# vita-epfl/motion-style-transfer

Hardware: AMD Instinct MI355X
Metric: trajectories/sec fwd+bwd (Y-Net+LoRA, SDD shortterm) (higher is better)
Workload: dtype f32; 1 GPU; C2: SDD shortterm Y-Net + LoRA rank=1 on encoder[0-4], 256x256 raster, obs=8 pred=12; batch_per_gpu=32, global_batch=32, raster=256x256, obs_len=8, pred_len=12, train_net=mosa_1, parallelism=dp1, trainable_floats=8190

## Files before the change

### motion-style-transfer_amd/csrc/wgrad_mfma.hip

```cpp
#include "ynet_common.h"
#include "../../include/ynet_hip.h"
#include <type_traits>
#include <stdlib.h>
#include <stdio.h>

struct WgradArgs {
    YSrc src[YNET_MAX_SRC];
    int nsrc, cin;
    const float* dy;
    long long dy_bs;
    const float* mask;
    long long mask_bs;
    float* partial_w;
    float* partial_b;
    int B, H, W, cout;
    int tiles_x, tiles_y, ntiles, nsplit, co_blks, ci_blks;
    int seg, nseg_y, nsegs;
    int debug;
#ifdef YNET_WG_PROFILE
    unsigned long long* prof;
#endif
};

template <int KS>
// ... 504 lines not shown
#endif
    for (; tile < a.ntiles; tile += a.nsplit) {
#ifdef YNET_WG_PROFILE
        const unsigned long long p0 = __builtin_amdgcn_s_memtime();
#endif
        asm volatile("s_waitcnt vmcnt(0)" ::: "memory");
#ifdef YNET_WG_PROFILE
        const unsigned long long p1 = __builtin_amdgcn_s_memtime();
#endif
        __syncthreads();
#ifdef YNET_WG_PROFILE
        const unsigned long long p2 = __builtin_amdgcn_s_memtime();
#endif
        if (tile + a.nsplit < a.ntiles) issue(next_tile(), buf ^ 1);
#ifdef YNET_WG_PROFILE
        const unsigned long long p3 = __builtin_amdgcn_s_memtime();
#endif
        compute(buf);
#ifdef YNET_WG_PROFILE
        const unsigned long long p4 = __builtin_amdgcn_s_memtime();
        pw += p1 - p0; pb += p2 - p1; pi += p3 - p2; pc += p4 - p3;
#endif
        buf ^= 1;
    }
#ifdef YNET_WG_PROFILE
    if (lane == 0) {
        unsigned long long* pr = a.prof;
        atomicAdd(pr + 0, __builtin_amdgcn_s_memtime() - pt0);
        atomicAdd(pr + 1, pw); atomicAdd(pr + 2, pb); atomicAdd(pr + 3, pi); atomicAdd(pr + 4, pc); atomicAdd(pr + 5, 1ull);
        atomicAdd(pr + 6, prof_dma);
    }
#endif

    if (rpN > 1) {
        float* red = smem;
        __syncthreads();
        if (rp > 0) {
            float* w = red + (wave - cbN * ibN) * 37 * 64 + lane;
#pragma unroll
            for (int t = 0; t < KK; ++t)
#pragma unroll
                for (int e = 0; e < 4; ++e) w[(t * 4 + e) * 64] = acc[t][e];
            w[36 * 64] = bsum;
        }
        __syncthreads();
        if (rp == 0) {
            for (int q = 1; q < rpN; ++q) {
                const float* w = red + (cb + cbN * (ib + ibN * q) - cbN * ibN) * 37 * 64 + lane;
#pragma unroll
                for (int t = 0; t < KK; ++t)
#pragma unroll
                    for (int e = 0; e < 4; ++e) acc[t][e] += w[(t * 4 + e) * 64];
                bsum += w[36 * 64];
            }
        }
    }
    if (rp == 0) {
        float* pw = a.partial_w + (long long)split * a.cout * a.cin * KK;
        const int ci = ib * 16 + r16;
#pragma unroll
        for (int e = 0; e < 4; ++e) {
            const int co = cb * 16 + 4 * kq + e;
            if (co < nco && ci < ncib) {
#pragma unroll
                for (int t = 0; t < KK; ++t) pw[((long long)(co0 + co) * a.cin + ci0 + ci) * KK + t] = acc[t][e];
            }
        }
        if (want_bias && ib == 0) {
            float v = bsum;
            v += __shfl_xor(v, 16);
            v += __shfl_xor(v, 32);
            const int co = cb * 16 + r16;
            if (kq == 0 && co < nco) a.partial_b[(long long)split * a.cout + co0 + co] = v;
        }
    }
}

typedef float f32x2 __attribute__((ext_vector_type(2)));
template <int OFF>
__device__ __forceinline__ void wg_ld2(f32x2& v, unsigned addr) {
    asm volatile("ds_read_b64 %0, %1 offset:%2" : "=v"(v) : "v"(addr), "n"(OFF));
}

template <bool MASK>
struct WgRollCfg {
    static constexpr int TW = 32, XCS = 44, XRS = 32 * XCS, XPS = 2 * XRS, XRING = 3 * XPS;
    static constexpr int PQ = 2 * 32 * 11;
    static constexpr int XI = (PQ + 255) / 256;
    static constexpr int DDATA = 2 * TW / 4, DQ = (DDATA + 1 + 6) / 8 * 8 + 1, DCH = DQ * 4;
    static constexpr int DS = 32 * DCH + 128, DBUF = DS * (MASK ? 2 : 1);
    static constexpr int DI = (32 * DQ + 255) / 256;
    static constexpr int LDS_FLOATS = XRING + 2 * DBUF, LDS_BYTES = LDS_FLOATS * 4;
    static constexpr int NGRP = 8;
    static_assert(DCH % 32 == 4 && (XCS * 4) % 16 == 0, "operand strides");
    static_assert(3 * 37 * 64 <= LDS_FLOATS, "cross-wave reduction scratch fits");
};

template <bool MASK>
__global__ __launch_bounds__(256, MASK ? 2 : 3) void wgrad_roll_kernel(const WgradArgs a) {
    using C = WgRollCfg<MASK>;
    constexpr int TW = C::TW, XCS = C::XCS, XRS = C::XRS, XPS = C::XPS, DQ = C::DQ, DCH = C::DCH, XI = C::XI, DI = C::DI, KK = 9;
    extern __shared__ __attribute__((aligned(16))) float smem[];
    auto ds_of = [&](int b) { return smem + C::XRING + b * C::DBUF; };
    auto ms_of = [&](int b) { return smem + C::XRING + b * C::DBUF + C::DS; };

    const int tid = threadIdx.x, lane = tid & 63;
    const int wave = __builtin_amdgcn_readfirstlane(tid >> 6);
    const int r16 = lane & 15, kq = lane >> 4;
    int bid = blockIdx.x;
    const int cib = bid % a.ci_blks;
    bid /= a.ci_blks;
    const int cob = bid % a.co_blks;
    const int split = bid / a.co_blks;
    const int H = a.H, W = a.W;
    const int HW = __builtin_amdgcn_readfirstlane(H * W);
    const unsigned plane_bytes = (unsigned)HW * 4u;
    const int ci0 = cib * 32, co0 = cob * 32;
    const int ncib = min(32, a.cin - ci0), nco = min(32, a.cout - co0);
    const bool want_bias = (a.partial_b != nullptr) && cib == 0;
    const int cbN = nco > 16 ? 2 : 1, ibN = ncib > 16 ? 2 : 1, rpN = 4 / (cbN * ibN);
    const int cb = wave % cbN, ib = (wave / cbN) % ibN, rp = wave / (cbN * ibN);

    int xsrc[XI], xrow[XI], xcol[XI];
    unsigned xcoff[XI];
#pragma unroll
    for (int k = 0; k < XI; ++k) {
        const int q = tid + k * 256;
        const int row = q / 352, within = q - row * 352, ch = within / 11, u = within - ch * 11;
        xrow[k] = row;
        xcol[k] = 4 * u - 4;
        int c = ci0 + ch, sid = -1;
        unsigned off = 0;
        if (q < C::PQ && u < 10 && ch < ncib) {
#pragma unroll
            for (int s = 0; s < YNET_MAX_SRC; ++s) {
                if (sid < 0 && s < a.nsrc) {
                    if (c < a.src[s].c) {
                        sid = s;
                        off = (unsigned)c * plane_bytes;
                    } else {
                        c -= a.src[s].c;
                    }
                }
            }
        }
        xsrc[k] = sid;
        xcoff[k] = off;
    }
    unsigned xs_in[XI], xs_l[XI], xs_r[XI], xs_lr[XI];
#pragma unroll
    for (int k = 0; k < XI; ++k) {
        const bool ok = xsrc[k] >= 0;
        const unsigned in = ok ? xcoff[k] + (unsigned)(xrow[k] * W + xcol[k] + 4) * 4u : 0x80000000u;
        const bool lh = xcol[k] < 0, rh = xcol[k] >= TW;
        xs_in[k] = in;
        xs_l[k] = lh ? 0x80000000u : in;
        xs_r[k] = rh ? 0x80000000u : in;
        xs_lr[k] = (lh || rh) ? 0x80000000u : in;
    }
    unsigned dstat[DI];
#pragma unroll
    for (int k = 0; k < DI; ++k) {
        const int q = tid + k * 256;
        const int ch = q / DQ, within = q - ch * DQ;
        const bool ok = q < 32 * DQ && within < C::DDATA;
        dstat[k] = ok ? (unsigned)ch * plane_bytes + (unsigned)((within / (TW / 4)) * W + (within % (TW / 4)) * 4) * 4u : 0x80000000u;
    }

    typedef const __attribute__((address_space(4))) WgradArgs* wg_kargs_t;
    auto issue_pair = [&](int b, int x0, int m, int slot) {
        wg_kargs_t ka = (wg_kargs_t)__builtin_amdgcn_kernarg_segment_ptr();
        asm volatile("" : "+s"(ka));
        float* xs = smem + slot * XPS;
        const int y0 = 2 * m - 1;
        const bool at_left = x0 == 0, at_right = x0 + TW >= W;
        unsigned xo[XI], xso;
        if (y0 >= 0 && y0 + 1 < H && y0 * W + x0 - 4 >= 0) {
            xso = (unsigned)(y0 * W + x0 - 4) * 4u;
            if (!at_left && !at_right) {
#pragma unroll
                for (int k = 0; k < XI; ++k) xo[k] = xs_in[k];
            } else {
#pragma unroll
                for (int k = 0; k < XI; ++k) {
                    const unsigned l = at_right ? xs_lr[k] : xs_l[k];
                    xo[k] = at_left ? l : xs_r[k];
                }
            }
        } else {
            xso = 0u;
#pragma unroll
            for (int k = 0; k < XI; ++k) {
                const int gy = y0 + xrow[k], gx = x0 + xcol[k];
                const bool ok = xsrc[k] >= 0 && gy >= 0 && gy < H && gx >= 0 && gx < W;
                xo[k] = ok ? xcoff[k] + (unsigned)(gy * W + gx) * 4u : 0x80000000u;
            }
        }
        const int nsrc = ka->nsrc;
        if (nsrc == 1) {
            const __amdgpu_buffer_rsrc_t r = __builtin_amdgcn_make_buffer_rsrc(
                const_cast<float*>(ka->src[0].p + (long long)b * ka->src[0].bs), 0, (unsigned)ka->src[0].c * plane_bytes, 0x00020000);
#pragma unroll
            for (int k = 0; k < XI - 1; ++k) wg_dma16s(r, xs + (k * 256 + wave * 64) * 4, xo[k], xso);
            if (wave < 3) wg_dma16s(r, xs + ((XI - 1) * 256 + wave * 64) * 4, xo[XI - 1], xso);
        } else {
#pragma unroll 1
            for (int s = 0; s < nsrc; ++s) {
                const __amdgpu_buffer_rsrc_t r = __builtin_amdgcn_make_buffer_rsrc(
                    const_cast<float*>(ka->src[s].p + (long long)b * ka->src[s].bs), 0, (unsigned)ka->src[s].c * plane_bytes, 0x00020000);
#pragma unroll
                for (int k = 0; k < XI; ++k)
                    if (xsrc[k] == s) wg_dma16s(r, xs + (k * 256 + wave * 64) * 4, xo[k], xso);
            }
        }
    };
    auto issue_dy = [&](int b, int x0, int j, int buf) {
        wg_kargs_t ka = (wg_kargs_t)__builtin_amdgcn_kernarg_segment_ptr();
        asm volatile("" : "+s"(ka));
        constexpr int DFULL = 32 * DQ / 256;
        static_assert(32 * DQ - DFULL * 256 <= 64, "the partial instruction fits one wave");
        const unsigned dso = (unsigned)(2 * j * W + x0) * 4u;
        {
            const __amdgpu_buffer_rsrc_t r = __builtin_amdgcn_make_buffer_rsrc(
                const_cast<float*>(ka->dy + (long long)b * ka->dy_bs + (long long)co0 * HW), 0, (unsigned)nco * plane_bytes, 0x00020000);
            float* ds = ds_of(buf);
#pragma unroll
            for (int k = 0; k < DFULL; ++k) wg_dma16s(r, ds + (k * 256 + wave * 64) * 4, dstat[k], dso);
            if (DI > DFULL && wave == 0) wg_dma16s(r, ds + (DFULL * 256) * 4, dstat[DI - 1], dso);
        }
        if (MASK) {
            const __amdgpu_buffer_rsrc_t r = __builtin_amdgcn_make_buffer_rsrc(
                const_cast<float*>(ka->mask + (long long)b * ka->mask_bs + (long long)co0 * HW), 0, (unsigned)nco * plane_bytes, 0x00020000);
            float* ms = ms_of(buf);
#pragma unroll
            for (int k = 0; k < DFULL; ++k) wg_dma16s(r, ms + (k * 256 + wave * 64) * 4, dstat[k], dso);
            if (DI > DFULL && wave == 0) wg_dma16s(r, ms + (DFULL * 256) * 4, dstat[DI - 1], dso);
        }
    };

    f32x4 acc[KK];
#pragma unroll
    for (int i = 0; i < KK; ++i) acc[i] = f32x4{0.f, 0.f, 0.f, 0.f};

    const unsigned x_lane = (unsigned)(size_t)(wg_lds_ptr_t)(smem + (ib * 16 + r16) * XCS + 2 * kq + 2) + 32u * rp;
    const unsigned d_lane = (unsigned)(size_t)(wg_lds_ptr_t)(smem + C::XRING + (cb * 16 + r16) * DCH + 2 * kq) + 32u * rp;
    f32x2 bsum2 = f32x2{0.f, 0.f};
    auto compute = [&](auto rpn_tag, int buf, unsigned sa, unsigned sb) {
        constexpr int RPN = decltype(rpn_tag)::value, NG = C::NGRP / RPN;
        const unsigned ab = d_lane + (unsigned)(buf * C::DBUF * 4), mb = ab + C::DS * 4;
        unsigned pa[4];
        pa[0] = x_lane + sa;
        pa[1] = x_lane + sa + XRS * 4;
        pa[2] = x_lane + sb;
        pa[3] = x_lane + sb + XRS * 4;
        f32x2 av[2], mv[2], q[2][KK];
        mv[0] = mv[1] = f32x2{1.f, 1.f};
        auto rd = [&](auto g_tag, f32x2& a_, f32x2& m_, f32x2* q_) {
            constexpr int G = decltype(g_tag)::value, r = G >> 2, col = (G & 3) * 32;
            wg_ld2<32 * G>(a_, ab);
            if (MASK) wg_ld2<32 * G>(m_, mb);
            wg_ld2<col>(q_[0], pa[r]);
            wg_ld2<col + 8>(q_[1], pa[r]);
            wg_ld2<col + 16>(q_[2], pa[r]);
            wg_ld2<col>(q_[3], pa[r + 1]);
            wg_ld2<col + 8>(q_[4], pa[r + 1]);
            wg_ld2<col + 16>(q_[5], pa[r + 1]);
            wg_ld2<col>(q_[6], pa[r + 2]);
            wg_ld2<col + 8>(q_[7], pa[r + 2]);
            wg_ld2<col + 16>(q_[8], pa[r + 2]);
        };
        auto lds_wait = []() { asm volatile("s_waitcnt lgkmcnt(0)" ::: "memory"); };
        auto select = [&](f32x2& a_, const f32x2& m_) {
            if (MASK) {
                a_.x = m_.x > 0.f ? a_.x : 0.f;
                a_.y = m_.y > 0.f ? a_.y : 0.f;
            }
        };
        auto mfmas = [&](const f32x2& a_c, const f32x2* q_c) {
#pragma unroll
            for (int ky = 0; ky < 3; ++ky) {
                acc[ky * 3 + 0] = __builtin_amdgcn_mfma_f32_16x16x4f32(a_c.x, q_c[ky * 3 + 0].y, acc[ky * 3 + 0], 0, 0, 0);
                acc[ky * 3 + 1] = __builtin_amdgcn_mfma_f32_16x16x4f32(a_c.x, q_c[ky * 3 + 1].x, acc[ky * 3 + 1], 0, 0, 0);
                acc[ky * 3 + 2] = __builtin_amdgcn_mfma_f32_16x16x4f32(a_c.x, q_c[ky * 3 + 1].y, acc[ky * 3 + 2], 0, 0, 0);
            }
#pragma unroll
            for (int ky = 0; ky < 3; ++ky) {
                acc[ky * 3 + 0] = __builtin_amdgcn_mfma_f32_16x16x4f32(a_c.y, q_c[ky * 3 + 1].x, acc[ky * 3 + 0], 0, 0, 0);
                acc[ky * 3 + 1] = __builtin_amdgcn_mfma_f32_16x16x4f32(a_c.y, q_c[ky * 3 + 1].y, acc[ky * 3 + 1], 0, 0, 0);
                acc[ky * 3 + 2] = __builtin_amdgcn_mfma_f32_16x16x4f32(a_c.y, q_c[ky * 3 + 2].x, acc[ky * 3 + 2], 0, 0, 0);
            }
        };
        rd(std::integral_constant<int, 0>{}, av[0], mv[0], q[0]);
        lds_wait();
        select(av[0], mv[0]);
        auto groups = [&](auto self, auto i_tag) -> void {
            constexpr int I = decltype(i_tag)::value, cur = I & 1, nxt = cur ^ 1;
#ifdef YNET_WG_EXPERIMENT
            if constexpr (I + 1 < NG) if (!(a.debug & 4)) rd(std::integral_constant<int, (I + 1) * RPN>{}, av[nxt], mv[nxt], q[nxt]);
#else
            if constexpr (I + 1 < NG) rd(std::integral_constant<int, (I + 1) * RPN>{}, av[nxt], mv[nxt], q[nxt]);
#endif
            __builtin_amdgcn_sched_barrier(0);
            mfmas(av[cur], q[cur]);
            __builtin_amdgcn_sched_barrier(0);
            if constexpr (I + 1 < NG) {
                lds_wait();
                select(av[nxt], mv[nxt]);
            }
            bsum2 += av[cur];
            __builtin_amdgcn_sched_barrier(0);
            if constexpr (I + 1 < NG) self(self, std::integral_constant<int, I + 1>{});
        };
        groups(groups, std::integral_constant<int, 0>{});
    };

    const int seg = a.seg, nseg_y = a.nseg_y, tiles_x = a.tiles_x, tiles_y = a.tiles_y;
    bool first = true;
    for (int sidx = split; sidx < a.nsegs; sidx += a.nsplit) {
        const int xt = sidx % tiles_x, t2 = sidx / tiles_x;
        const int ys = t2 % nseg_y, b = t2 / nseg_y;
        const int x0 = xt * TW, j0 = ys * seg, j1 = min(j0 + seg, tiles_y);
        if (!first) __syncthreads();
        first = false;
        issue_pair(b, x0, j0, 0);
        issue_pair(b, x0, j0 + 1, 1);
        issue_dy(b, x0, j0, 0);
        int sj = 0, buf = 0;
        for (int j = j0; j < j1; ++j) {
            asm volatile("s_waitcnt vmcnt(0)" ::: "memory");
            __syncthreads();
            const int s1 = sj == 2 ? 0 : sj + 1, s2 = s1 == 2 ? 0 : s1 + 1;
            if (j + 1 < j1 && !(a.debug & 1)) {
                issue_pair(b, x0, j + 2, s2);
                issue_dy(b, x0, j + 1, buf ^ 1);
            }
            if (!(a.debug & 2)) {
                const unsigned sa = (unsigned)(sj * XPS * 4), sb = (unsigned)(s1 * XPS * 4);
                if (rpN == 1) compute(std::integral_constant<int, 1>{}, buf, sa, sb);
                else if (rpN == 2) compute(std::integral_constant<int, 2>{}, buf, sa, sb);
                else compute(std::integral_constant<int, 4>{}, buf, sa, sb);
            }
            buf ^= 1;
            sj = s1;
        }
    }

    float bsum = bsum2.x + bsum2.y;
    if (rpN > 1) {
        float* red = smem;
        __syncthreads();
        if (rp > 0) {
            float* w = red + (wave - cbN * ibN) * 37 * 64 + lane;
#pragma unroll
            for (int t = 0; t < KK; ++t)
#pragma unroll
                for (int e = 0; e < 4; ++e) w[(t * 4 + e) * 64] = acc[t][e];
            w[36 * 64] = bsum2.x + bsum2.y;
        }
        __syncthreads();
        if (rp == 0) {
            for (int q = 1; q < rpN; ++q) {
                const float* w = red + (cb + cbN * (ib + ibN * q) - cbN * ibN) * 37 * 64 + lane;
#pragma unroll
                for (int t = 0; t < KK; ++t)
#pragma unroll
                    for (int e = 0; e < 4; ++e) acc[t][e] += w[(t * 4 + e) * 64];
                bsum += w[36 * 64];
            }
        }
    }
    if (rp == 0) {
        float* pw = a.partial_w + (long long)split * a.cout * a.cin * KK;
        const int ci = ib * 16 + r16;
#pragma unroll
        for (int e = 0; e < 4; ++e) {
            const int co = cb * 16 + 4 * kq + e;
            if (co < nco && ci < ncib) {
#pragma unroll
                for (int t = 0; t < KK; ++t) pw[((long long)(co0 + co) * a.cin + ci0 + ci) * KK + t] = acc[t][e];
            }
        }
        if (want_bias && ib == 0) {
            float v = bsum;
            v += __shfl_xor(v, 16);
            v += __shfl_xor(v, 32);
            const int co = cb * 16 + r16;
            if (kq == 0 && co < nco) a.partial_b[(long long)split * a.cout + co0 + co] = v;
        }
    }
}

struct Wg1x1Args {
    const float* x;
    long long x_bs;
    const float* dy;
    long long dy_bs;
    float* partial_w;
    float* partial_b;
    int B, cout, HW, hw16;
    long long chunks;
};

template <int CT>
__global__ __launch_bounds__(256) void wgrad1x1_stream_kernel(const Wg1x1Args a) {
    __shared__ float red[3][CT * 2 * 4 + CT][64];
    const int lane = threadIdx.x & 63, wave = threadIdx.x >> 6, r16 = lane & 15, kq = lane >> 4;
    f32x4 acc[CT][2];
    float bs[CT];
#pragma unroll
    for (int t = 0; t < CT; ++t) {
        acc[t][0] = acc[t][1] = f32x4{0.f, 0.f, 0.f, 0.f};
        bs[t] = 0.f;
    }
    const long long stride = (long long)gridDim.x * 4;
    long long c = (long long)blockIdx.x * 4 + wave;
    int b = (int)(c / a.hw16), pc = (int)(c - (long long)b * a.hw16);
    const int sb = (int)(stride / a.hw16), sp = (int)(stride - (long long)sb * a.hw16);
    const long long HW = a.HW;
    auto load = [&](int bb, int pp, f32x4& xa, f32x4& xb, f32x4* d) {
        const float* xp = a.x + (long long)bb * a.x_bs + (long long)r16 * HW + pp * 16 + 4 * kq;
        xa = *reinterpret_cast<const f32x4*>(xp);
        xb = *reinterpret_cast<const f32x4*>(xp + 16 * HW);
        const float* dp = a.dy + (long long)bb * a.dy_bs + (long long)r16 * HW + pp * 16 + 4 * kq;
#pragma unroll
        for (int t = 0; t < CT; ++t)
            d[t] = (t * 16 + r16 < a.cout) ? *reinterpret_cast<const f32x4*>(dp + (long long)t * 16 * HW) : f32x4{0.f, 0.f, 0.f, 0.f};
    };
    f32x4 xa, xb, d[CT], nxa, nxb, nd[CT];
    if (c < a.chunks) load(b, pc, xa, xb, d);
    while (c < a.chunks) {
        const long long cn = c + stride;
        int bn = b + sb, pn = pc + sp;
        if (pn >= a.hw16) {
            pn -= a.hw16;
            ++bn;
        }
        if (cn < a.chunks) load(bn, pn, nxa, nxb, nd);
#pragma unroll
        for (int e = 0; e < 4; ++e)
#pragma unroll
            for (int t = 0; t < CT; ++t) {
                acc[t][0] = __builtin_amdgcn_mfma_f32_16x16x4f32(d[t][e], xa[e], acc[t][0], 0, 0, 0);
                acc[t][1] = __builtin_amdgcn_mfma_f32_16x16x4f32(d[t][e], xb[e], acc[t][1], 0, 0, 0);
                bs[t] += d[t][e];
            }
        xa = nxa;
        xb = nxb;
#pragma unroll
        for (int t = 0; t < CT; ++t) d[t] = nd[t];
        c = cn;
        b = bn;
        pc = pn;
    }
    if (wave > 0) {
#pragma unroll
        for (int t = 0; t < CT; ++t) {
#pragma unroll
            for (int h = 0; h < 2; ++h)
#pragma unroll
                for (int e = 0; e < 4; ++e) red[wave - 1][(t * 2 + h) * 4 + e][lane] = acc[t][h][e];
// ... 101 lines not shown

template <bool MASK, int TH_>
static int launch_wgrad_dma(WgradArgs& a, float* dw, float* db, hipStream_t st) {
    using C = WgDmaCfg<MASK, TH_>;
    static bool attr_dev[YNET_MAX_DEV] = {false};
    bool& attr_set = attr_dev[ynet_device_slot()];
    if (!attr_set) {
        (void)hipFuncSetAttribute(reinterpret_cast<const void*>(wgrad_dma_kernel<MASK, TH_>),
                                  hipFuncAttributeMaxDynamicSharedMemorySize, 160 * 1024);
        attr_set = true;
        if (getenv("YNET_DEBUG_OCC")) {
            int per_cu = 0;
            (void)hipOccupancyMaxActiveBlocksPerMultiprocessor(&per_cu, wgrad_dma_kernel<MASK, TH_>, 256, C::LDS_BYTES);
            fprintf(stderr, "wgrad_dma_kernel<%d,%d>: %d bytes of LDS, %d workgroups per CU\n", (int)MASK, TH_, C::LDS_BYTES, per_cu);
        }
    }
    const long long nblk = (long long)a.nsplit * a.co_blks * a.ci_blks;
    static const bool timing = getenv("YNET_WGRAD_TIME") != nullptr;
    hipEvent_t e0 = nullptr, e1 = nullptr;
    if (timing) {
        (void)hipEventCreate(&e0);
        (void)hipEventCreate(&e1);
        (void)hipEventRecord(e0, st);
    }
#ifdef YNET_WG_PROFILE
    static unsigned long long* prof_dev = nullptr;
    if (!prof_dev) (void)hipMalloc(&prof_dev, 64);
    (void)hipMemsetAsync(prof_dev, 0, 64, st);
    a.prof = prof_dev;
#endif
    ynet_note_launch(1, 2);
    hipLaunchKernelGGL((wgrad_dma_kernel<MASK, TH_>), dim3((unsigned)nblk), dim3(256), C::LDS_BYTES, st, a);
#ifdef YNET_WG_PROFILE
    {
        unsigned long long h[8];
        (void)hipMemcpyAsync(h, prof_dev, 64, hipMemcpyDeviceToHost, st);
        (void)hipStreamSynchronize(st);
        const double tot = (double)h[0];
        fprintf(stderr, "wgrad_dma<%d> waves %llu avg cycles %.0f: vmcnt-wait %.1f%% barrier %.1f%% issue %.1f%% (of which DMA + descriptors %.1f%%) compute %.1f%% rest %.1f%%\n", (int)MASK,
                h[5], tot / (double)h[5], 100.0 * h[1] / tot, 100.0 * h[2] / tot, 100.0 * h[3] / tot, 100.0 * h[6] / tot, 100.0 * h[4] / tot,
                100.0 * (tot - h[1] - h[2] - h[3] - h[4]) / tot);
    }
#endif
    if (timing) {
        (void)hipEventRecord(e1, st);
        (void)hipEventSynchronize(e1);
        float ms = 0.f;
        (void)hipEventElapsedTime(&ms, e0, e1);
        fprintf(stderr, "wgrad_dma_kernel<%d> B %d %dx%d cin %d cout %d nsplit %d tiles %d blocks %lld: %.1f us  %.1f TFLOP/s\n", (int)MASK, a.B, a.H, a.W,
                a.cin, a.cout, a.nsplit, a.ntiles, nblk, ms * 1e3f, 2.0 * a.B * a.H * a.W * (double)a.cin * a.cout * 9 / (ms * 1e9));
        (void)hipEventDestroy(e0);
        (void)hipEventDestroy(e1);
    }
    int rc = ynet_check_launch("conv2d_wgrad");
    if (rc) return rc;
    const long long nw = (long long)a.cout * a.cin * 9;
    launch_reduce_partials(a, dw, db, nw, st);
    return ynet_check_launch("conv2d_wgrad(reduce)");
}

static int launch_wgrad1x1_stream(WgradArgs& a, int ct, float* dw, float* db, hipStream_t st) {
    Wg1x1Args k{};
    k.x = a.src[0].p;
    k.x_bs = a.src[0].bs;
    k.dy = a.dy;
    k.dy_bs = a.dy_bs;
    k.B = a.B;
    k.cout = a.cout;
    k.HW = a.H * a.W;
    k.hw16 = k.HW / 16;
    k.chunks = (long long)a.B * k.hw16;
    const int grid = a.nsplit;
    k.partial_w = a.partial_w;
    k.partial_b = a.partial_b;
    ynet_note_launch(1, 4);
    if (ct == 1) hipLaunchKernelGGL(wgrad1x1_stream_kernel<1>, dim3(grid), dim3(256), 0, st, k);
    else hipLaunchKernelGGL(wgrad1x1_stream_kernel<2>, dim3(grid), dim3(256), 0, st, k);
    int rc = ynet_check_launch("conv2d_wgrad(1x1)");
    if (rc) return rc;
    launch_reduce_partials(a, dw, db, (long long)a.cout * 32, st);
    return ynet_check_launch("conv2d_wgrad(reduce)");
}

template <bool MASK>
static int launch_wgrad_roll(WgradArgs& a, float* dw, float* db, hipStream_t st) {
    using C = WgRollCfg<MASK>;
    static bool attr_dev[YNET_MAX_DEV] = {false};
    bool& attr_set = attr_dev[ynet_device_slot()];
    if (!attr_set) {
        (void)hipFuncSetAttribute(reinterpret_cast<const void*>(wgrad_roll_kernel<MASK>), hipFuncAttributeMaxDynamicSharedMemorySize, 160 * 1024);
        attr_set = true;
        if (getenv("YNET_DEBUG_OCC")) {
            int per_cu = 0;
            (void)hipOccupancyMaxActiveBlocksPerMultiprocessor(&per_cu, wgrad_roll_kernel<MASK>, 256, C::LDS_BYTES);
            fprintf(stderr, "wgrad_roll_kernel<%d>: %d bytes of LDS, %d workgroups per CU\n", (int)MASK, C::LDS_BYTES, per_cu);
        }
    }
    const long long nblk = (long long)a.nsplit * a.co_blks * a.ci_blks;
    static const bool timing = getenv("YNET_WGRAD_TIME") != nullptr;
    hipEvent_t e0 = nullptr, e1 = nullptr;
    if (timing) {
        (void)hipEventCreate(&e0);
        (void)hipEventCreate(&e1);
        (void)hipEventRecord(e0, st);
    }
    ynet_note_launch(1, 3);
    hipLaunchKernelGGL((wgrad_roll_kernel<MASK>), dim3((unsigned)nblk), dim3(256), C::LDS_BYTES, st, a);
    if (timing) {
        (void)hipEventRecord(e1, st);
        (void)hipEventSynchronize(e1);
        float ms = 0.f;
        (void)hipEventElapsedTime(&ms, e0, e1);
        fprintf(stderr, "wgrad_roll_kernel<%d> B %d %dx%d cin %d cout %d nsplit %d segments %d x %d steps, blocks %lld: %.1f us  %.1f TFLOP/s\n", (int)MASK, a.B,
                a.H, a.W, a.cin, a.cout, a.nsplit, a.nsegs, a.seg, nblk, ms * 1e3f, 2.0 * a.B * a.H * a.W * (double)a.cin * a.cout * 9 / (ms * 1e9));
        (void)hipEventDestroy(e0);
        (void)hipEventDestroy(e1);
    }
    int rc = ynet_check_launch("conv2d_wgrad");
    if (rc) return rc;
    launch_reduce_partials(a, dw, db, (long long)a.cout * a.cin * 9, st);
    return ynet_check_launch("conv2d_wgrad(reduce)");
}

static bool wgrad_roll_plan(YnetWgradPlan& p, int B, int H, int W, int cin, bool masked) {
    static const int on = getenv("YNET_WGRAD_ROLL") ? atoi(getenv("YNET_WGRAD_ROLL")) : 1;
    static const int forced = getenv("YNET_WGRAD_SEG") ? atoi(getenv("YNET_WGRAD_SEG")) : 0;
    if (!on || (W % 32) != 0 || (H & 1) != 0) return false;
    const int tiles_y = H / 2, strips = B * (W / 32);
    int nsplit = p.nsplit;
    static const int wg3 = getenv("YNET_WGRAD_WG3") ? atoi(getenv("YNET_WGRAD_WG3")) : 1;
    if (!masked && wg3) {
        const int blocks = p.co_blks * ceil_div(cin, 32);
        int n = 768 / blocks;
        if (n < 1) n = 1;
        if (n > p.ntiles) n = p.ntiles;
        nsplit = n;
    }
    int seg = 0;
    for (int s : {16, 8, 4})
        if (seg == 0 && (long long)strips * ceil_div(tiles_y, s) >= 3ll * nsplit) seg = s;
    if (seg == 0 && (long long)strips * ceil_div(tiles_y, 4) >= nsplit) seg = 4;
    if (forced > 0) seg = forced;
    if (seg == 0 || tiles_y < 2) return false;
    p.seg = seg;
    p.nseg_y = ceil_div(tiles_y, seg);
    p.nsegs = strips * p.nseg_y;
    p.nsplit = nsplit > p.nsegs ? p.nsegs : nsplit;
    return true;
}

static int wgrad_roll_debug() {
    static const int debug = getenv("YNET_WGRAD_DEBUG") ? atoi(getenv("YNET_WGRAD_DEBUG")) : 0;
    return debug;
}

template <int KS>
static int launch_wgrad(WgradArgs& a, float* dw, float* db, hipStream_t st) {
    static_assert(WgCfg<KS>::CIB == (KS == 5 ? 6 : 32), "wgrad_cib: the plan's input-channel block is the kernel's");
    return a.mask ? launch_wgrad_m<KS, true>(a, dw, db, st) : launch_wgrad_m<KS, false>(a, dw, db, st);
}

static int wgrad_cib(int K) { return K == 5 ? 6 : 32; }

static bool wgrad_dma_shape(int W, int K) {
    static const int on = getenv("YNET_WGRAD_DMA") ? atoi(getenv("YNET_WGRAD_DMA")) : 1;
    return on && K == 3 && (W % 4) == 0;
}

static int wgrad_plan(int B, int H, int W, int cout, int cin, int K, int th, int* nsplit_out) {
    const int tiles = B * ceil_div(H, th) * ceil_div(W, 32);
    const int blocks_per_split = ceil_div(cout, 32) * ceil_div(cin, wgrad_cib(K));
    const int resident = th == 1 ? 768 : 512;
    int nsplit = resident / blocks_per_split;
    if (nsplit < 1) nsplit = 1;
    if (nsplit > tiles) nsplit = tiles;
    if (nsplit > resident) nsplit = resident;
    *nsplit_out = nsplit;
    return tiles;
}

static const int WG1X1_BLOCKS = 512;
static bool wgrad1x1_stream_ok(int H, int W, int cout, int cin, int nsrc, int K, bool masked, bool aligned) {
    static const int on = getenv("YNET_WGRAD_1X1_STREAM") ? atoi(getenv("YNET_WGRAD_1X1_STREAM")) : 1;
    return on && K == 1 && nsrc == 1 && cin == 32 && cout <= 32 && !masked && ((long long)H * W) % 16 == 0 && aligned;
}

static void wgrad_fill_plan(int B, int H, int W, int cout, int cin, int nsrc, int K, bool masked, bool aligned, bool want_bias, YnetWgradPlan& p) {
    p = YnetWgradPlan{};
    const bool dma = wgrad_dma_shape(W, K) && aligned;
    const int th = dma ? 2 : 4;
    p.rows = th;
    p.tiles_x = ceil_div(W, 32);
    p.tiles_y = ceil_div(H, th);
    p.ntiles = wgrad_plan(B, H, W, cout, cin, K, th, &p.nsplit);
    p.co_blks = ceil_div(cout, 32);
    p.ci_blks = ceil_div(cin, wgrad_cib(K));
    if (dma) {
        p.kernel = wgrad_roll_plan(p, B, H, W, cin, masked) ? 3 : 2;
    } else if (wgrad1x1_stream_ok(H, W, cout, cin, nsrc, K, masked, aligned)) {
        p.kernel = 4;
        p.rows = 0;
        const long long chunks = (long long)B * (((long long)H * W) / 16);
        int grid = WG1X1_BLOCKS;
        if ((long long)grid * 4 > chunks) grid = (int)((chunks + 3) / 4);
        p.nsplit = grid;
        p.ct = cout <= 16 ? 1 : 2;
    } else {
        p.kernel = 1;
    }
    p.partial_floats = (long long)p.nsplit * cout * cin * K * K + (want_bias ? (long long)p.nsplit * cout : 0);
}

extern "C" {

long long ynet_conv2d_wgrad_workspace_floats(int B, int H, int W, int cout, int cin, int K) {
    int n1 = 0, n2 = 0, n4 = 0;
    wgrad_plan(B, H, W, cout, cin, K, 1, &n1);
    wgrad_plan(B, H, W, cout, cin, K, 2, &n2);
    wgrad_plan(B, H, W, cout, cin, K, 4, &n4);
    int n = n1 > n2 ? (n1 > n4 ? n1 : n4) : (n2 > n4 ? n2 : n4);
    if (K == 1 && n < WG1X1_BLOCKS) n = WG1X1_BLOCKS;
    return (long long)n * ((long long)cout * cin * K * K + cout);
}

int ynet_conv2d_wgrad(const float* const* src, const int* src_c, const long long* src_bs, int nsrc,
                      const float* dy, long long dy_bs, const float* mask, long long mask_bs,
                      float* dw, float* db, float* workspace, int B, int H, int W, int cout, int K,
                      void* stream) {
    YNET_REQUIRE(nsrc >= 1 && nsrc <= YNET_MAX_SRC, "conv2d_wgrad: 1..%d sources supported", YNET_MAX_SRC);
    YNET_REQUIRE(dy && dw && workspace, "conv2d_wgrad: null pointer");
    YNET_REQUIRE(B > 0 && H > 0 && W > 0 && cout > 0, "conv2d_wgrad: empty problem");
    WgradArgs a{};
    a.nsrc = nsrc;
    a.cin = 0;
    for (int i = 0; i < nsrc; ++i) {
        YNET_REQUIRE(src[i] != nullptr && src_c[i] > 0, "conv2d_wgrad: source %d is null/empty", i);
        a.src[i] = YSrc{src[i], src_c[i], src_bs[i], 0};
        a.cin += src_c[i];
    }
    a.dy = dy;
    a.dy_bs = dy_bs;
    a.mask = mask;
    a.mask_bs = mask_bs;
    a.B = B;
    a.H = H;
    a.W = W;
    a.cout = cout;
    bool aligned = true;
    {
        auto misaligned = [](const void* p, long long bs) { return (reinterpret_cast<uintptr_t>(p) & 15) != 0 || (bs & 3) != 0; };
        for (int i = 0; i < nsrc; ++i) aligned = aligned && !misaligned(src[i], src_bs[i]);
        aligned = aligned && !misaligned(dy, dy_bs) && (mask == nullptr || !misaligned(mask, mask_bs));
    }
    YnetWgradPlan p;
    wgrad_fill_plan(B, H, W, cout, a.cin, nsrc, K, mask != nullptr, aligned, db != nullptr, p);
    a.tiles_x = p.tiles_x;
    a.tiles_y = p.tiles_y;
    a.ntiles = p.ntiles;
    a.nsplit = p.nsplit;
    a.co_blks = p.co_blks;
    a.ci_blks = p.ci_blks;
    a.seg = p.seg;
    a.nseg_y = p.nseg_y;
    a.nsegs = p.nsegs;
    a.partial_w = workspace;
    a.partial_b = db ? workspace + (long long)a.nsplit * cout * a.cin * K * K : nullptr;
    hipStream_t st = (hipStream_t)stream;
    switch (p.kernel) {
        case 3:
            a.debug = wgrad_roll_debug();
            return mask ? launch_wgrad_roll<true>(a, dw, db, st) : launch_wgrad_roll<false>(a, dw, db, st);
        case 2: return mask ? launch_wgrad_dma<true, 2>(a, dw, db, st) : launch_wgrad_dma<false, 2>(a, dw, db, st);
        case 4: return launch_wgrad1x1_stream(a, p.ct, dw, db, st);
        default: break;
    }
    switch (K) {
        case 1: return launch_wgrad<1>(a, dw, db, st);
        case 3: return launch_wgrad<3>(a, dw, db, st);
        case 5: return launch_wgrad<5>(a, dw, db, st);
        default: ynet_set_error("conv2d_wgrad: kernel size %d not supported (1, 3, 5)", K); return 1;
    }
}

int ynet_conv2d_wgrad_plan(int B, int H, int W, int cout, const int* src_c, int nsrc, int K, int masked, int aligned, int want_bias,
                           YnetWgradPlan* out) {
    YNET_REQUIRE(out != nullptr && src_c != nullptr, "conv2d_wgrad_plan: null pointer");
    YNET_REQUIRE(nsrc >= 1 && nsrc <= YNET_MAX_SRC, "conv2d_wgrad_plan: 1..%d sources supported", YNET_MAX_SRC);
    YNET_REQUIRE(B > 0 && H > 0 && W > 0 && cout > 0, "conv2d_wgrad_plan: empty problem");
    YNET_REQUIRE(K == 1 || K == 3 || K == 5, "conv2d_wgrad_plan: kernel size %d not supported (1, 3, 5)", K);
    int cin = 0;
    for (int i = 0; i < nsrc; ++i) {
        YNET_REQUIRE(src_c[i] > 0, "conv2d_wgrad_plan: source %d is empty", i);
        cin += src_c[i];
    }
    wgrad_fill_plan(B, H, W, cout, cin, nsrc, K, masked != 0, aligned != 0, want_bias != 0, *out);
    return 0;
}

}
```

Baseline: 4987 trajectories/s.

## Add narrow-channel forms to rolling 3x3 wgrad kernel with flattened tap accumulators

Adds two specialised forms of the rolling-window 3x3 weight-gradient kernel for layers with at most 16 input channels. Both halve the input ring to 16 channels with a padded row stride, which shrinks LDS use. For 14 or fewer channels, a flat form packs (channel, tap) pairs into 16-wide MFMA columns, so it needs 8 accumulators instead of 9 and does no MFMA work on empty channel slots. This comes at the cost of per-lane gathered LDS addresses, split 32-bit reads, and a loop unrolled three ways over ring phases.

Result: no change. 5004 trajectories/s (median of 6 runs) (+0.3%).

```diff
diff --git a/motion-style-transfer_amd/csrc/wgrad_mfma.hip b/motion-style-transfer_amd/csrc/wgrad_mfma.hip
--- a/motion-style-transfer_amd/csrc/wgrad_mfma.hip
+++ b/motion-style-transfer_amd/csrc/wgrad_mfma.hip
@@ -610,24 +610,41 @@
     asm volatile("ds_read_b64 %0, %1 offset:%2" : "=v"(v) : "v"(addr), "n"(OFF));
 }
 
-template <bool MASK>
+template <bool MASK, int FORM>
 struct WgRollCfg {
-    static constexpr int TW = 32, XCS = 44, XRS = 32 * XCS, XPS = 2 * XRS, XRING = 3 * XPS;
-    static constexpr int PQ = 2 * 32 * 11;
+    static constexpr bool NARROW = FORM != 0, FLAT = FORM == 2;
+    static constexpr int TW = 32, XCS = 44, XCH = NARROW ? 16 : 32;
+    static constexpr int XRS = XCH * XCS + (NARROW ? 23 * 4 : 0);
+    static constexpr int PQ = XRS / 4 + XCH * 11;
     static constexpr int XI = (PQ + 255) / 256;
+    static constexpr int XLASTW = (PQ - (XI - 1) * 256 + 63) / 64;
+    static constexpr int XPS = 2 * XRS, XRING = 3 * XPS;
+    static constexpr int NACC = FLAT ? 8 : 9, RED = NACC * 4 + 1;
+    static_assert(XRS % 4 == 0 && ((XI - 1) * 256 + XLASTW * 64) * 4 <= XPS, "a pair's DMA (whole waves) stays inside its ring slot");
+    static_assert(!NARROW || XRS % 32 == 28, "narrow ring: consecutive rows 28 banks apart");
     static constexpr int DDATA = 2 * TW / 4, DQ = (DDATA + 1 + 6) / 8 * 8 + 1, DCH = DQ * 4;
     static constexpr int DS = 32 * DCH + 128, DBUF = DS * (MASK ? 2 : 1);
     static constexpr int DI = (32 * DQ + 255) / 256;
     static constexpr int LDS_FLOATS = XRING + 2 * DBUF, LDS_BYTES = LDS_FLOATS * 4;
     static constexpr int NGRP = 8;
     static_assert(DCH % 32 == 4 && (XCS * 4) % 16 == 0, "operand strides");
-    static_assert(3 * 37 * 64 <= LDS_FLOATS, "cross-wave reduction scratch fits");
+    static_assert(3 * RED * 64 <= LDS_FLOATS, "cross-wave reduction scratch fits");
 };
 
-template <bool MASK>
+template <int OFF>
+__device__ __forceinline__ void wg_ld11(f32x2& v, unsigned addr) {
+    float lo, hi;
+    asm volatile("ds_read_b32 %0, %1 offset:%2" : "=v"(lo) : "v"(addr), "n"(OFF));
+    asm volatile("ds_read_b32 %0, %1 offset:%2" : "=v"(hi) : "v"(addr), "n"(OFF + 4));
+    v = f32x2{lo, hi};
+}
+
+template <bool MASK, int FORM>
 __global__ __launch_bounds__(256, MASK ? 2 : 3) void wgrad_roll_kernel(const WgradArgs a) {
-    using C = WgRollCfg<MASK>;
+    using C = WgRollCfg<MASK, FORM>;
     constexpr int TW = C::TW, XCS = C::XCS, XRS = C::XRS, XPS = C::XPS, DQ = C::DQ, DCH = C::DCH, XI = C::XI, DI = C::DI, KK = 9;
+    constexpr int NACC = C::NACC, ROWQ = XRS / 4;
+    constexpr bool FLAT = C::FLAT;
     extern __shared__ __attribute__((aligned(16))) float smem[];
     auto ds_of = [&](int b) { return smem + C::XRING + b * C::DBUF; };
     auto ms_of = [&](int b) { return smem + C::XRING + b * C::DBUF + C::DS; };
@@ -654,12 +671,12 @@
 #pragma unroll
     for (int k = 0; k < XI; ++k) {
         const int q = tid + k * 256;
-        const int row = q / 352, within = q - row * 352, ch = within / 11, u = within - ch * 11;
+        const int row = q / ROWQ, within = q - row * ROWQ, ch = within / 11, u = within - ch * 11;
         xrow[k] = row;
         xcol[k] = 4 * u - 4;
         int c = ci0 + ch, sid = -1;
         unsigned off = 0;
-        if (q < C::PQ && u < 10 && ch < ncib) {
+        if (q < C::PQ && u < 10 && ch < C::XCH && ch < ncib) {
 #pragma unroll
             for (int s = 0; s < YNET_MAX_SRC; ++s) {
                 if (sid < 0 && s < a.nsrc) {
@@ -730,7 +747,7 @@
                 const_cast<float*>(ka->src[0].p + (long long)b * ka->src[0].bs), 0, (unsigned)ka->src[0].c * plane_bytes, 0x00020000);
 #pragma unroll
             for (int k = 0; k < XI - 1; ++k) wg_dma16s(r, xs + (k * 256 + wave * 64) * 4, xo[k], xso);
-            if (wave < 3) wg_dma16s(r, xs + ((XI - 1) * 256 + wave * 64) * 4, xo[XI - 1], xso);
+            if (wave < C::XLASTW) wg_dma16s(r, xs + ((XI - 1) * 256 + wave * 64) * 4, xo[XI - 1], xso);
         } else {
 #pragma unroll 1
             for (int s = 0; s < nsrc; ++s) {
@@ -766,36 +783,56 @@
         }
     };
 
-    f32x4 acc[KK];
-#pragma unroll
-    for (int i = 0; i < KK; ++i) acc[i] = f32x4{0.f, 0.f, 0.f, 0.f};
+    f32x4 acc[NACC];
+#pragma unroll
+    for (int i = 0; i < NACC; ++i) acc[i] = f32x4{0.f, 0.f, 0.f, 0.f};
 
     const unsigned x_lane = (unsigned)(size_t)(wg_lds_ptr_t)(smem + (ib * 16 + r16) * XCS + 2 * kq + 2) + 32u * rp;
     const unsigned d_lane = (unsigned)(size_t)(wg_lds_ptr_t)(smem + C::XRING + (cb * 16 + r16) * DCH + 2 * kq) + 32u * rp;
     f32x2 bsum2 = f32x2{0.f, 0.f};
-    auto compute = [&](auto rpn_tag, int buf, unsigned sa, unsigned sb) {
-        constexpr int RPN = decltype(rpn_tag)::value, NG = C::NGRP / RPN;
+    unsigned xa[FLAT ? NACC : 1][FLAT ? 3 : 1];
+    if constexpr (FLAT) {
+        const int ncol = KK * ncib;
+#pragma unroll
+        for (int t = 0; t < NACC; ++t) {
+            const int u = min(16 * t + r16, ncol - 1), ci = u / KK, tap = u - ci * KK, ky = tap / 3, kx = tap - 3 * ky;
+            const unsigned g = (unsigned)(size_t)(wg_lds_ptr_t)(smem + ci * XCS + 2 * kq + 3 + kx) + 32u * rp;
+            xa[t][0] = g + (unsigned)(ky * XRS * 4);
+            xa[t][1] = g + (unsigned)(((4 + ky) % 6) * XRS * 4);
+            xa[t][2] = g + (unsigned)(((5 + ky) % 6) * XRS * 4);
+        }
+    }
+    auto compute = [&](auto rpn_tag, auto ph_tag, int buf, unsigned sa, unsigned sb) {
+        constexpr int RPN = decltype(rpn_tag)::value, NG = C::NGRP / RPN, PH = decltype(ph_tag)::value;
         const unsigned ab = d_lane + (unsigned)(buf * C::DBUF * 4), mb = ab + C::DS * 4;
         unsigned pa[4];
         pa[0] = x_lane + sa;
         pa[1] = x_lane + sa + XRS * 4;
         pa[2] = x_lane + sb;
         pa[3] = x_lane + sb + XRS * 4;
-        f32x2 av[2], mv[2], q[2][KK];
+        f32x2 av[2], mv[2], q[2][NACC];
         mv[0] = mv[1] = f32x2{1.f, 1.f};
         auto rd = [&](auto g_tag, f32x2& a_, f32x2& m_, f32x2* q_) {
             constexpr int G = decltype(g_tag)::value, r = G >> 2, col = (G & 3) * 32;
             wg_ld2<32 * G>(a_, ab);
             if (MASK) wg_ld2<32 * G>(m_, mb);
-            wg_ld2<col>(q_[0], pa[r]);
-            wg_ld2<col + 8>(q_[1], pa[r]);
-            wg_ld2<col + 16>(q_[2], pa[r]);
-            wg_ld2<col>(q_[3], pa[r + 1]);
-            wg_ld2<col + 8>(q_[4], pa[r + 1]);
-            wg_ld2<col + 16>(q_[5], pa[r + 1]);
-            wg_ld2<col>(q_[6], pa[r + 2]);
-            wg_ld2<col + 8>(q_[7], pa[r + 2]);
-            wg_ld2<col + 16>(q_[8], pa[r + 2]);
+            if constexpr (FLAT) {
+#pragma unroll
+                for (int t = 0; t < NACC; ++t) {
+                    constexpr int c = 2 * PH + r;
+                    wg_ld11<col + (c <= 3 ? c * XRS * 4 : 0)>(q_[t], xa[t][c <= 3 ? 0 : c - 3]);
+                }
+            } else {
+                wg_ld2<col>(q_[0], pa[r]);
+                wg_ld2<col + 8>(q_[1], pa[r]);
+                wg_ld2<col + 16>(q_[2], pa[r]);
+                wg_ld2<col>(q_[3], pa[r + 1]);
+                wg_ld2<col + 8>(q_[4], pa[r + 1]);
+                wg_ld2<col + 16>(q_[5], pa[r + 1]);
+                wg_ld2<col>(q_[6], pa[r + 2]);
+                wg_ld2<col + 8>(q_[7], pa[r + 2]);
+                wg_ld2<col + 16>(q_[8], pa[r + 2]);
+            }
         };
         auto lds_wait = []() { asm volatile("s_waitcnt lgkmcnt(0)" ::: "memory"); };
         auto select = [&](f32x2& a_, const f32x2& m_) {
@@ -805,17 +842,24 @@
             }
         };
         auto mfmas = [&](const f32x2& a_c, const f32x2* q_c) {
-#pragma unroll
-            for (int ky = 0; ky < 3; ++ky) {
-                acc[ky * 3 + 0] = __builtin_amdgcn_mfma_f32_16x16x4f32(a_c.x, q_c[ky * 3 + 0].y, acc[ky * 3 + 0], 0, 0, 0);
-                acc[ky * 3 + 1] = __builtin_amdgcn_mfma_f32_16x16x4f32(a_c.x, q_c[ky * 3 + 1].x, acc[ky * 3 + 1], 0, 0, 0);
-                acc[ky * 3 + 2] = __builtin_amdgcn_mfma_f32_16x16x4f32(a_c.x, q_c[ky * 3 + 1].y, acc[ky * 3 + 2], 0, 0, 0);
-            }
-#pragma unroll
-            for (int ky = 0; ky < 3; ++ky) {
-                acc[ky * 3 + 0] = __builtin_amdgcn_mfma_f32_16x16x4f32(a_c.y, q_c[ky * 3 + 1].x, acc[ky * 3 + 0], 0, 0, 0);
-                acc[ky * 3 + 1] = __builtin_amdgcn_mfma_f32_16x16x4f32(a_c.y, q_c[ky * 3 + 1].y, acc[ky * 3 + 1], 0, 0, 0);
-                acc[ky * 3 + 2] = __builtin_amdgcn_mfma_f32_16x16x4f32(a_c.y, q_c[ky * 3 + 2].x, acc[ky * 3 + 2], 0, 0, 0);
+            if constexpr (FLAT) {
+#pragma unroll
+                for (int t = 0; t < NACC; ++t) acc[t] = __builtin_amdgcn_mfma_f32_16x16x4f32(a_c.x, q_c[t].x, acc[t], 0, 0, 0);
+#pragma unroll
+                for (int t = 0; t < NACC; ++t) acc[t] = __builtin_amdgcn_mfma_f32_16x16x4f32(a_c.y, q_c[t].y, acc[t], 0, 0, 0);
+            } else {
+#pragma unroll
+                for (int ky = 0; ky < 3; ++ky) {
+                    acc[ky * 3 + 0] = __builtin_amdgcn_mfma_f32_16x16x4f32(a_c.x, q_c[ky * 3 + 0].y, acc[ky * 3 + 0], 0, 0, 0);
+                    acc[ky * 3 + 1] = __builtin_amdgcn_mfma_f32_16x16x4f32(a_c.x, q_c[ky * 3 + 1].x, acc[ky * 3 + 1], 0, 0, 0);
+                    acc[ky * 3 + 2] = __builtin_amdgcn_mfma_f32_16x16x4f32(a_c.x, q_c[ky * 3 + 1].y, acc[ky * 3 + 2], 0, 0, 0);
+                }
+#pragma unroll
+                for (int ky = 0; ky < 3; ++ky) {
+                    acc[ky * 3 + 0] = __builtin_amdgcn_mfma_f32_16x16x4f32(a_c.y, q_c[ky * 3 + 1].x, acc[ky * 3 + 0], 0, 0, 0);
+                    acc[ky * 3 + 1] = __builtin_amdgcn_mfma_f32_16x16x4f32(a_c.y, q_c[ky * 3 + 1].y, acc[ky * 3 + 1], 0, 0, 0);
+                    acc[ky * 3 + 2] = __builtin_amdgcn_mfma_f32_16x16x4f32(a_c.y, q_c[ky * 3 + 2].x, acc[ky * 3 + 2], 0, 0, 0);
+                }
             }
         };
         rd(std::integral_constant<int, 0>{}, av[0], mv[0], q[0]);
@@ -843,57 +887,86 @@
     };
 
     const int seg = a.seg, nseg_y = a.nseg_y, tiles_x = a.tiles_x, tiles_y = a.tiles_y;
-    bool first = true;
-    for (int sidx = split; sidx < a.nsegs; sidx += a.nsplit) {
-        const int xt = sidx % tiles_x, t2 = sidx / tiles_x;
-        const int ys = t2 % nseg_y, b = t2 / nseg_y;
-        const int x0 = xt * TW, j0 = ys * seg, j1 = min(j0 + seg, tiles_y);
-        if (!first) __syncthreads();
-        first = false;
-        issue_pair(b, x0, j0, 0);
-        issue_pair(b, x0, j0 + 1, 1);
-        issue_dy(b, x0, j0, 0);
-        int sj = 0, buf = 0;
-        for (int j = j0; j < j1; ++j) {
-            asm volatile("s_waitcnt vmcnt(0)" ::: "memory");
-            __syncthreads();
-            const int s1 = sj == 2 ? 0 : sj + 1, s2 = s1 == 2 ? 0 : s1 + 1;
-            if (j + 1 < j1 && !(a.debug & 1)) {
-                issue_pair(b, x0, j + 2, s2);
-                issue_dy(b, x0, j + 1, buf ^ 1);
-            }
-            if (!(a.debug & 2)) {
-                const unsigned sa = (unsigned)(sj * XPS * 4), sb = (unsigned)(s1 * XPS * 4);
-                if (rpN == 1) compute(std::integral_constant<int, 1>{}, buf, sa, sb);
-                else if (rpN == 2) compute(std::integral_constant<int, 2>{}, buf, sa, sb);
-                else compute(std::integral_constant<int, 4>{}, buf, sa, sb);
-            }
-            buf ^= 1;
-            sj = s1;
-        }
-    }
+    auto walk = [&](auto rpn_flat) {
+        bool first = true;
+        for (int sidx = split; sidx < a.nsegs; sidx += a.nsplit) {
+            const int xt = sidx % tiles_x, t2 = sidx / tiles_x;
+            const int ys = t2 % nseg_y, b = t2 / nseg_y;
+            const int x0 = xt * TW, j0 = ys * seg, j1 = min(j0 + seg, tiles_y);
+            if (!first) __syncthreads();
+            first = false;
+            issue_pair(b, x0, j0, 0);
+            issue_pair(b, x0, j0 + 1, 1);
+            issue_dy(b, x0, j0, 0);
+            int buf = 0;
+            if constexpr (!FLAT) {
+                constexpr std::integral_constant<int, 0> ph0{};
+                int sj = 0;
+                for (int j = j0; j < j1; ++j) {
+                    asm volatile("s_waitcnt vmcnt(0)" ::: "memory");
+                    __syncthreads();
+                    const int s1 = sj == 2 ? 0 : sj + 1, s2 = s1 == 2 ? 0 : s1 + 1;
+                    if (j + 1 < j1 && !(a.debug & 1)) {
+                        issue_pair(b, x0, j + 2, s2);
+                        issue_dy(b, x0, j + 1, buf ^ 1);
+                    }
+                    if (!(a.debug & 2)) {
+                        const unsigned sa = (unsigned)(sj * XPS * 4), sb = (unsigned)(s1 * XPS * 4);
+                        if (rpN == 1) compute(std::integral_constant<int, 1>{}, ph0, buf, sa, sb);
+                        else if (rpN == 2) compute(std::integral_constant<int, 2>{}, ph0, buf, sa, sb);
+                        else compute(std::integral_constant<int, 4>{}, ph0, buf, sa, sb);
+                    }
+                    buf ^= 1;
+                    sj = s1;
+                }
+            } else {
+                auto step = [&](auto ph_tag, int j) {
+                    constexpr int S2 = (decltype(ph_tag)::value + 2) % 3;
+                    asm volatile("s_waitcnt vmcnt(0)" ::: "memory");
+                    __syncthreads();
+                    if (j + 1 < j1 && !(a.debug & 1)) {
+                        issue_pair(b, x0, j + 2, S2);
+                        issue_dy(b, x0, j + 1, buf ^ 1);
+                    }
+                    compute(rpn_flat, ph_tag, buf, 0u, 0u);
+                    buf ^= 1;
+                };
+                for (int j = j0; j < j1;) {
+                    step(std::integral_constant<int, 0>{}, j);
+                    if (++j >= j1) break;
+                    step(std::integral_constant<int, 1>{}, j);
+                    if (++j >= j1) break;
+                    step(std::integral_constant<int, 2>{}, j);
+                    ++j;
+                }
+            }
+        }
+    };
+    if constexpr (!FLAT) walk(std::integral_constant<int, 1>{});
+    else if (rpN == 2) walk(std::integral_constant<int, 2>{});
+    else walk(std::integral_constant<int, 4>{});
 
     float bsum = bsum2.x + bsum2.y;
     if (rpN > 1) {
         float* red = smem;
         __syncthreads();
         if (rp > 0) {
-            float* w = red + (wave - cbN * ibN) * 37 * 64 + lane;
-#pragma unroll
-            for (int t = 0; t < KK; ++t)
+            float* w = red + (wave - cbN * ibN) * C::RED * 64 + lane;
+#pragma unroll
+            for (int t = 0; t < NACC; ++t)
 #pragma unroll
                 for (int e = 0; e < 4; ++e) w[(t * 4 + e) * 64] = acc[t][e];
-            w[36 * 64] = bsum2.x + bsum2.y;
+            w[NACC * 4 * 64] = bsum2.x + bsum2.y;
         }
         __syncthreads();
         if (rp == 0) {
             for (int q = 1; q < rpN; ++q) {
-                const float* w = red + (cb + cbN * (ib + ibN * q) - cbN * ibN) * 37 * 64 + lane;
-#pragma unroll
-                for (int t = 0; t < KK; ++t)
+                const float* w = red + (cb + cbN * (ib + ibN * q) - cbN * ibN) * C::RED * 64 + lane;
+#pragma unroll
+                for (int t = 0; t < NACC; ++t)
 #pragma unroll
                     for (int e = 0; e < 4; ++e) acc[t][e] += w[(t * 4 + e) * 64];
-                bsum += w[36 * 64];
+                bsum += w[NACC * 4 * 64];
             }
         }
     }
@@ -903,7 +976,11 @@
 #pragma unroll
         for (int e = 0; e < 4; ++e) {
             const int co = cb * 16 + 4 * kq + e;
-            if (co < nco && ci < ncib) {
+            if constexpr (FLAT) {
+#pragma unroll
+                for (int t = 0; t < NACC; ++t)
+                    if (co < nco && 16 * t + r16 < KK * ncib) pw[(long long)(co0 + co) * a.cin * KK + 16 * t + r16] = acc[t][e];
+            } else if (co < nco && ci < ncib) {
 #pragma unroll
                 for (int t = 0; t < KK; ++t) pw[((long long)(co0 + co) * a.cin + ci0 + ci) * KK + t] = acc[t][e];
             }
@@ -1171,18 +1248,18 @@
     return ynet_check_launch("conv2d_wgrad(reduce)");
 }
 
-template <bool MASK>
+template <bool MASK, int FORM>
 static int launch_wgrad_roll(WgradArgs& a, float* dw, float* db, hipStream_t st) {
-    using C = WgRollCfg<MASK>;
+    using C = WgRollCfg<MASK, FORM>;
     static bool attr_dev[YNET_MAX_DEV] = {false};
     bool& attr_set = attr_dev[ynet_device_slot()];
     if (!attr_set) {
-        (void)hipFuncSetAttribute(reinterpret_cast<const void*>(wgrad_roll_kernel<MASK>), hipFuncAttributeMaxDynamicSharedMemorySize, 160 * 1024);
+        (void)hipFuncSetAttribute(reinterpret_cast<const void*>(wgrad_roll_kernel<MASK, FORM>), hipFuncAttributeMaxDynamicSharedMemorySize, 160 * 1024);
         attr_set = true;
         if (getenv("YNET_DEBUG_OCC")) {
             int per_cu = 0;
-            (void)hipOccupancyMaxActiveBlocksPerMultiprocessor(&per_cu, wgrad_roll_kernel<MASK>, 256, C::LDS_BYTES);
-            fprintf(stderr, "wgrad_roll_kernel<%d>: %d bytes of LDS, %d workgroups per CU\n", (int)MASK, C::LDS_BYTES, per_cu);
+            (void)hipOccupancyMaxActiveBlocksPerMultiprocessor(&per_cu, wgrad_roll_kernel<MASK, FORM>, 256, C::LDS_BYTES);
+            fprintf(stderr, "wgrad_roll_kernel<%d, %d>: %d bytes of LDS, %d workgroups per CU\n", (int)MASK, FORM, C::LDS_BYTES, per_cu);
         }
     }
     const long long nblk = (long long)a.nsplit * a.co_blks * a.ci_blks;
@@ -1194,13 +1271,13 @@
         (void)hipEventRecord(e0, st);
     }
     ynet_note_launch(1, 3);
-    hipLaunchKernelGGL((wgrad_roll_kernel<MASK>), dim3((unsigned)nblk), dim3(256), C::LDS_BYTES, st, a);
+    hipLaunchKernelGGL((wgrad_roll_kernel<MASK, FORM>), dim3((unsigned)nblk), dim3(256), C::LDS_BYTES, st, a);
     if (timing) {
         (void)hipEventRecord(e1, st);
         (void)hipEventSynchronize(e1);
         float ms = 0.f;
         (void)hipEventElapsedTime(&ms, e0, e1);
-        fprintf(stderr, "wgrad_roll_kernel<%d> B %d %dx%d cin %d cout %d nsplit %d segments %d x %d steps, blocks %lld: %.1f us  %.1f TFLOP/s\n", (int)MASK, a.B,
+        fprintf(stderr, "wgrad_roll_kernel<%d, %d> B %d %dx%d cin %d cout %d nsplit %d segments %d x %d steps, blocks %lld: %.1f us  %.1f TFLOP/s\n", (int)MASK, FORM, a.B,
                 a.H, a.W, a.cin, a.cout, a.nsplit, a.nsegs, a.seg, nblk, ms * 1e3f, 2.0 * a.B * a.H * a.W * (double)a.cin * a.cout * 9 / (ms * 1e9));
         (void)hipEventDestroy(e0);
         (void)hipEventDestroy(e1);
@@ -1236,6 +1313,20 @@
     p.nsegs = strips * p.nseg_y;
     p.nsplit = nsplit > p.nsegs ? p.nsegs : nsplit;
     return true;
+}
+
+static int wgrad_roll_form(int cin) {
+    static const int on = getenv("YNET_WGRAD_NARROW") ? atoi(getenv("YNET_WGRAD_NARROW")) : 1;
+    return (!on || cin > 16) ? 0 : cin > 14 ? 1 : 2;
+}
+
+template <bool MASK>
+static int launch_wgrad_roll_form(WgradArgs& a, float* dw, float* db, hipStream_t st) {
+    switch (wgrad_roll_form(a.cin)) {
+        case 2: return launch_wgrad_roll<MASK, 2>(a, dw, db, st);
+        case 1: return launch_wgrad_roll<MASK, 1>(a, dw, db, st);
+        default: return launch_wgrad_roll<MASK, 0>(a, dw, db, st);
+    }
 }
 
 static int wgrad_roll_debug() {
@@ -1358,7 +1449,7 @@
     switch (p.kernel) {
         case 3:
             a.debug = wgrad_roll_debug();
-            return mask ? launch_wgrad_roll<true>(a, dw, db, st) : launch_wgrad_roll<false>(a, dw, db, st);
+            return mask ? launch_wgrad_roll_form<true>(a, dw, db, st) : launch_wgrad_roll_form<false>(a, dw, db, st);
         case 2: return mask ? launch_wgrad_dma<true, 2>(a, dw, db, st) : launch_wgrad_dma<false, 2>(a, dw, db, st);
         case 4: return launch_wgrad1x1_stream(a, p.ct, dw, db, st);
         default: break;
```
